# shidanxu/DistributedLPSolver

Hardware: AMD Instinct MI355X
Metric: simplex pivots/s + achieved HBM GB/s (dense fp64 tableau; roofline of the rank-64 tableau pass) (higher is better)
Workload: dtype f64

## Files before the change

distributedlpsolver_amd/csrc/dlp_defer.hip:

```cpp
#include <hip/hip_runtime.h>

#include <cmath>
#include <cstdlib>
#include <utility>

#include "dlp_internal.h"

namespace dlp {
namespace {

#include "dlp_device.h"

typedef unsigned int u4v __attribute__((ext_vector_type(4)));
typedef unsigned int u2v __attribute__((ext_vector_type(2)));
__device__ __forceinline__ u2v dbits(double v) {
    uint64_t u;
    __builtin_memcpy(&u, &v, sizeof(u));
    u2v w;
    w.x = (unsigned)u;
    w.y = (unsigned)(u >> 32);
    return w;
}

template <bool NT>
__device__ inline d2 ldv(const double* p) {
    if constexpr (NT)
        return __builtin_nontemporal_load((const d2*)p);
    else
        return *(const d2*)p;
}
template <bool NT>
__device__ inline double ldv1(const double* p) {
    if constexpr (NT)
        return __builtin_nontemporal_load(p);
    else
        return *p;
}
template <bool NT>
__device__ inline void stv1(double* p, double v) {
    if constexpr (NT)
        __builtin_nontemporal_store(v, p);
    else
        *p = v;
}
template <bool NT>
__device__ inline void stv(double* p, d2 v) {
    if constexpr (NT)
        __builtin_nontemporal_store(v, (d2*)p);
    else
        *(d2*)p = v;
}

__device__ __forceinline__ void glds16(const void* g, uint32_t m0) {
    asm volatile("s_waitcnt lgkmcnt(0)\n\tglobal_load_lds_dwordx4 %0, off" ::"v"(g), "{m0}"(m0) : "memory");
}
template <int N>
__device__ __forceinline__ void vmwait() { asm volatile("s_waitcnt vmcnt(%0)" ::"n"(N) : "memory"); }
__device__ __forceinline__ uint32_t lds_addr(const void* p) {
    return __builtin_amdgcn_readfirstlane((uint32_t)(uintptr_t)(const __attribute__((address_space(3))) void*)p);
}

constexpr int kAuxSc1 = 16;

__device__ inline void release_go(DevState* st) {
    __builtin_amdgcn_fence(__ATOMIC_RELEASE, "agent");
    asm volatile("s_waitcnt vmcnt(0)" ::: "memory");
    __hip_atomic_store(&st->go, 1u, __ATOMIC_RELAXED, __HIP_MEMORY_SCOPE_AGENT);
}

__device__ uint64_t g_chain_stamps[64][16];
__device__ int g_chain_stamps_on;
#define CHAIN_STAMP(slot, k)                                                                  \
    do {                                                                                      \
        if (g_chain_stamps_on && threadIdx.x == 0) g_chain_stamps[(slot) & 63][k] = wall_clock64(); \
    } while (0)
__device__ uint64_t g_wg_stamps[1024][8];
#define WG_STAMP(slot, k, v)                                                                   \
    do {                                                                                       \
        if (g_chain_stamps_on && threadIdx.x == 0 && ((slot) & 63) == 40 && blockIdx.x < 1024) \
            g_wg_stamps[blockIdx.x][k] = (v);                                                  \
    } while (0)

constexpr int kRatioRingPairs = 8;
constexpr size_t ratio_ring_bytes(int rp) { return (size_t)(kRatioDeferThreads / 64) * rp * 128 * sizeof(double); }
template <int KMAX, bool FUSED, bool LEAN = false, int LCH = 4, int RP = kRatioRingPairs, bool DB = false,
          int ROWS = 64, int RG = 1>
__device__ __forceinline__ void ratio_defer_body(
    const double* __restrict__ T, int64_t ld, int64_t rows, int64_t rows_elig, int64_t ncols,
    int64_t row_first, int32_t* basis, const PricePart* __restrict__ pp, int ntiles,
    DevState* st, double* __restrict__ C, int64_t ldc, double* __restrict__ Cc, int64_t ldcc,
    const double* __restrict__ P, double* __restrict__ rhs, int32_t* __restrict__ nzc,
    Cand* partials, Cand* cand_out, int nranks, double tol_dj, double tol_piv, int pricing,
    dlp_pivot* log, int64_t log_cap, int nblocks, const double* __restrict__ Ccp = nullptr,
    const double* __restrict__ Pp = nullptr, int prev_seal = -1, const XPeers* xp = nullptr,
    uint32_t xseq = 0, uint32_t* bcnt = nullptr, int brb = 1, int bnt = 0, const double* Tn = nullptr,
    int xsel = 0, uint32_t rseq = 0, Cond cd = Cond{}) {
    constexpr bool GRING = ROWS != 64 || RG != 1;
    constexpr int kPad = GRING ? 128 / ROWS * (RG + 1) : 0;
    constexpr int kWaves = GRING ? 16 : kRatioDeferThreads / 64;
    __shared__ PricePart lds_pp[kWaves];
    __shared__ Cand lds_c[kWaves];
    __shared__ int s_last;
    __shared__ double s_pq[KMAX + kPad], s_pn[KMAX];
    __shared__ int32_t s_pl[KMAX + kPad];
    auto cand_red = [&](Cand v) { return block_cand(v, lds_c); };
    const PricePart pp0 = (int)threadIdx.x < ntiles ? pp[threadIdx.x] : pp_empty();
    if (st->status != DLP_RUNNING) return;
// ... 1709 lines not shown
        vmwait<2 * U * (D - 1)>();
        return;
    }
    switch (g) {
        case 0: vmwait<U * (D - 1)>(); break;
        case 1: vmwait<U * (D - 1) + U>(); break;
        case 2: vmwait<U * (D - 1) + 2 * U>(); break;
        case 3: vmwait<U * (D - 1) + 3 * U>(); break;
        case 4: vmwait<U * (D - 1) + 4 * U>(); break;
        case 5: vmwait<U * (D - 1) + 5 * U>(); break;
        default: vmwait<U * (D - 1) + 6 * U>(); break;
    }
}
template <int U, int L>
__device__ __forceinline__ void ring_step(double (&t)[U], const double (&c)[U][2], const double (&pr)[64]) {
    constexpr int e = L & 1, n = (L & 31) >> 1;
#pragma unroll
    for (int u = 0; u < U; ++u) fmac_bc<n>(t[u], c[u][e], pr[L]);
}
template <int U, int L0, int... I>
__device__ __forceinline__ void ring_half(double (&t)[U], const double (&c)[U][2], const double (&pr)[64],
                                          std::integer_sequence<int, I...>) {
    (ring_step<U, L0 + I>(t, c, pr), ...);
}

template <int L>
__device__ __forceinline__ void redo_step(double& t, const double (&c)[2], const double (&pr)[64], int cl) {
    constexpr int e = L & 1, n = (L & 31) >> 1;
    if (L == cl)
        t = pr[L];
    else if (L > cl)
        fmac_bc<n>(t, c[e], pr[L]);
}
template <int L0, int... I>
__device__ __forceinline__ void redo_half(double& t, const double (&c)[2], const double (&pr)[64], int cl,
                                          std::integer_sequence<int, I...>) {
    (redo_step<L0 + I>(t, c, pr, cl), ...);
}
__device__ __forceinline__ double redo_pivot_row(const double* cr, int cl, const double (&pr)[64]) {
    int lane;
    asm volatile("v_mbcnt_lo_u32_b32 %0, -1, 0\n\tv_mbcnt_hi_u32_b32 %0, -1, %0" : "=v"(lane));
    double t = 0.0;
    if (cl < 32) {
        const d2 v = *(const d2*)(cr + 2 * (lane & 15));
        const double c0[2] = {v.x, v.y};
        redo_half<0>(t, c0, pr, cl, std::make_integer_sequence<int, 32>{});
    }
    const d2 v = *(const d2*)(cr + 32 + 2 * (lane & 15));
    const double c1[2] = {v.x, v.y};
    redo_half<32>(t, c1, pr, cl, std::make_integer_sequence<int, 32>{});
    return t;
}

template <bool NT, int U, int D, bool PUB = false>
__global__ __launch_bounds__(256) __attribute__((amdgpu_waves_per_eu(3))) void pass_q_kernel(
                                                     const double* __restrict__ T, double* __restrict__ Tout,
                                                     int64_t ld, int64_t rows, int64_t width,
                                                     const BlockDesc* __restrict__ bd,
                                                     const double* __restrict__ C, int64_t ldc,
                                                     const double* __restrict__ P,
                                                     const int32_t* __restrict__ nzc, int rb,
                                                     uint32_t* bcnt = nullptr, int pivg = 0) {
    constexpr int K = 64, SLOT = 128 * U;
    constexpr int kSt = (NT ? 2 : 0) | (PUB ? kAuxSc1 : 0);
    static_assert(U % 2 == 0, "one DMA carries two rows");
    __shared__ __attribute__((aligned(16))) int32_t cls[1024];
    typedef int32_t clsv __attribute__((ext_vector_type(U)));
    extern __shared__ double ring[];
    const int kb = bd->blk;
    const bool outplace = Tout != T;
    if (kb == 0 && !outplace) return;
    const int lane = threadIdx.x & 63;
    const int w = __builtin_amdgcn_readfirstlane(threadIdx.x >> 6);
    const int64_t j = (int64_t)blockIdx.x * 256 + threadIdx.x;
    const bool colok = j < width;
    const int jc = (int)(colok ? j : width - 1);
    double pr[K];
#pragma unroll
    for (int l = 0; l < K; ++l) pr[l] = P[(int64_t)l * ld + jc];
    const int64_t i0 = (int64_t)blockIdx.y * rb;
    const int64_t iend = (i0 + rb < rows) ? i0 + rb : rows;
    const int nr = (int)(iend - i0);
    classify_band(cls, bd, nzc, i0, nr, kb, pivg != 0);
    __syncthreads();
#pragma unroll
    for (int l = 0; l < K; ++l) asm volatile("" ::"v"(pr[l]));
    const int ng = (nr + U - 1) / U;
    const int64_t wc = (int64_t)blockIdx.x * 256 + w * 64 + 2 * (lane & 31);
    const int64_t wcc = wc < ld - 1 ? wc : ld - 2;
    const double* tsrc = T + i0 * ld + wcc;
    const double* csrc = C + i0 * ldc + 2 * (lane & 31);
    double* wbase = ring + (size_t)w * D * SLOT;
    const uint32_t lbase = (uint32_t)(uintptr_t)(const __attribute__((address_space(3))) void*)wbase;
    auto dma = [&](int g, int s) {
        const int gg = g < ng ? g : ng - 1;
#pragma unroll
        for (int k = 0; k < U / 2; ++k) {
            int r = gg * U + 2 * k + (lane >> 5);
            r = r < nr ? r : nr - 1;
            glds16(tsrc + (int64_t)r * ld, __builtin_amdgcn_readfirstlane(lbase + s * SLOT * 8 + k * 1024));
        }
#pragma unroll
        for (int k = 0; k < U / 2; ++k) {
            int r = gg * U + 2 * k + (lane >> 5);
            r = r < nr ? r : nr - 1;
            glds16(csrc + (int64_t)r * ldc,
                   __builtin_amdgcn_readfirstlane(lbase + s * SLOT * 8 + U * 512 + k * 1024));
        }
    };
    const int ld8 = (int)(ld * 8);
    const __amdgpu_buffer_rsrc_t ro = __builtin_amdgcn_make_buffer_rsrc(
        (void*)(Tout + i0 * ld), (short)0, (int)((int64_t)nr * ld * 8), 0x00020000);
    const int voff_st = colok ? jc * 8 : 0x7fffff00;
    auto store = [&](double v, int r, bool keep) {
        __builtin_amdgcn_raw_buffer_store_b64(__builtin_bit_cast(u2v, v), ro, keep ? voff_st : 0x7fffff00,
                                              (r < nr ? r : 0) * ld8, kSt);
    };
#pragma unroll
    for (int s = 0; s < D; ++s) dma(s, s);
    int s = 0;
    for (int g = 0; g < ng; ++g) {
        vmwait_group<D, U>(g);
        const double* sl = wbase + s * SLOT;
        const int r0 = g * U;
        const clsv cv = *(const clsv*)(cls + r0);
        bool dense = r0 + U <= nr, anyp = false;
#pragma unroll
        for (int u = 0; u < U; ++u) {
            const int cu = __builtin_amdgcn_readfirstlane(cv[u]);
            dense = dense && (cu == kDense || cu >= kDensePiv);
            anyp = anyp || cu >= kDensePiv;
        }
        if (dense) {
            double t[U];
#pragma unroll
            for (int u = 0; u < U; ++u) t[u] = sl[u * 64 + lane];
            double c[U][2];
            auto loadc = [&](int h) {
#pragma unroll
                for (int u = 0; u < U; ++u) {
                    const d2 v = *(const d2*)(sl + U * 64 + u * 64 + h * 32 + 2 * (lane & 15));
                    c[u][0] = v.x;
                    c[u][1] = v.y;
                }
            };
            loadc(0);
            ring_half<U, 0>(t, c, pr, std::make_integer_sequence<int, 32>{});
            loadc(1);
            ring_half<U, 32>(t, c, pr, std::make_integer_sequence<int, 32>{});
            if (anyp) {
#pragma nounroll
                for (int u = 0; u < U; ++u) {
                    const int cl = __builtin_amdgcn_readfirstlane(cls[r0 + u]) - kDensePiv;
                    if (cl < 0) continue;
                    const double tp = redo_pivot_row(sl + U * 64 + u * 64, cl, pr);
#pragma unroll
                    for (int k = 0; k < U; ++k) t[k] = k == u ? tp : t[k];
                }
            }
#pragma unroll
            for (int u = 0; u < U; ++u) store(t[u], r0 + u, true);
        } else {
            for (int u = 0; u < U; ++u) {
                const int r = r0 + u;
                int cl = r < nr ? cls[r] : kUntouched;
                if (cl >= kDensePiv) cl -= kDensePiv;
                double t = sl[u * 64 + lane];
                if (cl == kUntouched) {
                    store(t, r, outplace && r < nr);
                    continue;
                }
                const double* cr = sl + U * 64 + u * 64;
                t = replay_row(t, cl, pr, [&](int l) { return cr[l]; });
                store(t, r, true);
            }
        }
        dma(g + D, s);
        s = s + 1 == D ? 0 : s + 1;
    }
    if constexpr (PUB) {
        vmwait<0>();
        __syncthreads();
        if (threadIdx.x == 0) __hip_atomic_fetch_add(&bcnt[blockIdx.y], 1u, __ATOMIC_RELAXED, __HIP_MEMORY_SCOPE_AGENT);
    }
}


typedef double d4 __attribute__((ext_vector_type(4)));
template <bool NT_, int NT, bool PUB = false>
__global__ __launch_bounds__(256, 2) void pass_m_kernel(const double* __restrict__ T, double* __restrict__ Tout,
                                                     int64_t ld, int64_t rows, int64_t width,
                                                     const BlockDesc* __restrict__ bd,
                                                     const double* __restrict__ C, int64_t ldc,
                                                     const double* __restrict__ P,
                                                     const int32_t* __restrict__ nzc, int rb,
                                                     uint32_t* bcnt = nullptr) {
    constexpr int kSt = (NT_ ? 2 : 0) | (PUB ? kAuxSc1 : 0);
    constexpr int K = 64, KB = K / 4, W = 16 * NT, RS = K + 2;
    constexpr int NPC = (16 * RS + 127) / 128;
    __shared__ double lds_all[2 * NPC * 128 + 512];
    double(*As)[NPC * 128] = reinterpret_cast<double(*)[NPC * 128]>(lds_all);
    int32_t* cls = reinterpret_cast<int32_t*>(lds_all + 2 * NPC * 128);
    const int kb = bd->blk;
    const bool outplace = Tout != T;
    if (kb == 0 && !outplace) return;
    const int lane = threadIdx.x & 63;
    const int w = __builtin_amdgcn_readfirstlane(threadIdx.x >> 6);
    const int lr = lane & 15, lq = lane >> 4;
    const int64_t cw = (int64_t)blockIdx.x * (4 * W);
    const int64_t c0 = cw + w * W;
    double b[KB][NT];
#pragma unroll
    for (int k4 = 0; k4 < KB; ++k4)
#pragma unroll
        for (int t = 0; t < NT; ++t) {
            const int64_t col = c0 + 16 * t + lr;
            b[k4][t] = P[(int64_t)(4 * k4 + lq) * ld + (col < width ? col : width - 1)];
        }
    const int64_t i0 = (int64_t)blockIdx.y * rb;
    const int64_t iend = (i0 + rb < rows) ? i0 + rb : rows;
    const int nr = (int)(iend - i0);
    classify_band(cls, bd, nzc, i0, nr, kb);
    const int ng = (nr + 15) / 16;
    const int ld8 = (int)(ld * 8);
    const __amdgpu_buffer_rsrc_t ro = __builtin_amdgcn_make_buffer_rsrc(
        (void*)(Tout + i0 * ld), (short)0, (int)((int64_t)nr * ld * 8), 0x00020000);
    (void)ro;
    (void)ld8;
    auto stage = [&](int g, int buf) {
        const int gg = g < ng ? g : ng - 1;
// ... 93 lines not shown
                l = cl + 1;
            } else {
                t = row[j];
            }
            const double* cr = C + (i0 + r) * ldc;
            for (; l < kb; ++l) {
                const double f = cr[l];
                if (f != 0.0) t = __builtin_fma(-f, P[(int64_t)l * ld + j], t);
            }
        }
        if constexpr (PUB)
            __builtin_amdgcn_raw_buffer_store_b64(__builtin_bit_cast(u2v, t), ro, (int)j * 8 + r * ld8, 0, kSt);
        else
            Tout[(i0 + r) * ld + j] = t;
    }
    if constexpr (PUB) {
        asm volatile("s_waitcnt vmcnt(0)" ::: "memory");
        __syncthreads();
        if (threadIdx.x == 0) __hip_atomic_fetch_add(&bcnt[blockIdx.y], 1u, __ATOMIC_RELAXED, __HIP_MEMORY_SCOPE_AGENT);
    }
}

__global__ void blk_reset_kernel(DevState* st) {
    if (threadIdx.x == 0) {
        st->blk = 0;
        st->bser = st->bser + 1;
    }
}

__global__ __launch_bounds__(256) void reset_cols_kernel(double* __restrict__ T, int64_t ld, int64_t rows,
                                                         const int32_t* __restrict__ blkp,
                                                         const int32_t* __restrict__ pl,
                                                         const int32_t* __restrict__ qs) {
    const int64_t i = (int64_t)blockIdx.x * blockDim.x + threadIdx.x;
    if (i >= rows) return;
    const int kb = *blkp;
    double* r = T + i * ld;
    for (int l = 0; l < kb; ++l) r[qs[l]] = (pl[l] == (int32_t)i) ? 1.0 : 0.0;
}

__global__ __launch_bounds__(256) void drop_failed_step_kernel(const DevState* __restrict__ st,
                                                               const int32_t* __restrict__ blkp,
                                                               double* __restrict__ C, int64_t ldc,
                                                               int32_t* __restrict__ nzc, int64_t rows) {
    if (st->status != DLP_UNBOUNDED) return;
    const int kb = *blkp;
    const int64_t i = (int64_t)blockIdx.x * blockDim.x + threadIdx.x;
    if (i > rows || kb < 0 || kb >= ldc) return;
    const double a = C[i * ldc + kb];
    if (i < rows && a != 0.0) nzc[i] = nzc[i] - 1;
    C[i * ldc + kb] = 0.0;
}

__global__ __launch_bounds__(64) void seal_kernel(DevState* st, int slot, uint32_t* bcnt, int64_t nb) {
    const int kb = st->blk;
    for (int l = threadIdx.x; l < kMaxDefer; l += 64) {
        st->seal[slot].pl[l] = l < kb ? st->pl[l] : -1;
        st->seal[slot].qs[l] = st->qs[l];
    }
    if (bcnt)
        for (int64_t b = threadIdx.x; b < nb; b += 64) bcnt[b] = 0;
    __syncthreads();
    if (threadIdx.x == 0) {
        st->seal[slot].blk = kb;
        st->seal[slot].ser = st->bser;
        st->blk = 0;
        st->bser = st->bser + 1;
    }
}

}

static int ratio_ring_rows(const Geometry& g) {
    return g.rthreads >= 256 ? 64 : 0;
}

int ratio_defer_blocks(const Geometry& g) {
    return (int)((g.rows + 1 + g.rthreads - 1) / g.rthreads);
}
static int ratio_blocks_256(const Geometry& g) {
    return (int)((g.rows + 1 + kRatioDeferThreads - 1) / kRatioDeferThreads);
}

hipError_t launch_ratio_defer(const Geometry& g, const Defer& d, int32_t* basis,
                              const PricePart* pp, DevState* st, Cand* partials, int nblocks,
                              Cand* cand_out, int nranks, double tol_dj, double tol_piv,
                              int pricing, dlp_pivot* log, int64_t log_cap, hipStream_t s,
                              const Defer* prev, int prev_seal, const XPeers* xp, uint32_t xseq,
                              const BandPub* bp, bool xfuse, bool own_cus) {
    const int ntiles = (int)((g.width + kDeferTile - 1) / kDeferTile);
    const bool pub = bp && bp->cnt && bp->Tn && prev_seal >= 0;
    xfuse = xfuse && xp && nranks > 1;
    if (nblocks < ratio_defer_blocks(g)) return hipErrorInvalidValue;
    nblocks = ratio_defer_blocks(g);
    if (prev_seal >= 0 && (!prev || prev_seal > 1 || 2 * d.K > kMaxReplay)) return hipErrorInvalidValue;
    const double* Ccp = prev_seal >= 0 ? prev->Cc : nullptr;
    const double* Pp = prev_seal >= 0 ? prev->P : nullptr;
    const int steps = prev_seal >= 0 ? 2 * d.K : d.K;
    if (g.rthreads != 64 && g.rthreads != 128 && g.rthreads != 256) return hipErrorInvalidValue;
#define DLP_RATIO_DEFER(KM)                                                                      \
    ratio_defer_kernel<KM><<<nblocks, g.rthreads, 0, s>>>(                               \
        g.T, g.ld, g.rows, g.rows_elig, g.ncols, g.row_first, basis, pp, ntiles, st, d.C, d.ldc, \
        d.Cc, d.ldcc, d.P, d.rhs, d.nzc, partials, cand_out, nranks, tol_dj, tol_piv, pricing,   \
        log, log_cap, Ccp, Pp, prev_seal, xp, xseq, xfuse ? 1 : 0, g.cd)
    if (steps <= 8)
        DLP_RATIO_DEFER(8);
    else if (steps <= 16)
        DLP_RATIO_DEFER(16);
// ... 169 lines not shown
    g.T, g.ld, g.rows, g.rows_elig, g.ncols, g.nprice, g.row_first, basis, pp, ntiles, st, d.C, d.ldc, d.Cc, \
        d.ldcc, d.P, d.rhs, d.nzc, nrat, tol_dj, tol_piv, pricing, log, log_cap, Ccp, Pp, Cp, prev_seal, xp, \
        seq, pub ? bp->cnt + prev_seal * bp->stride : nullptr, pub ? bp->rb : 1, pub ? bp->ntiles : 0,     \
        pub ? bp->Tn : nullptr, 2, g.cd
    if (!ring && steps > 64 && g.cd.on) return hipErrorInvalidValue;
    if (ring) {
        if (g.rthreads == 128)
            pivot_x_ring_kernel<32><<<nrat + nprow, 256, (size_t)4 * 16 * 1024, s>>>(DLP_PX_ARGS);
        else
            pivot_x_ring_kernel<64><<<nrat + nprow, 256, (size_t)4 * 16 * 1024, s>>>(DLP_PX_ARGS);
    } else if (steps > 64)
        pivot_x_lean_kernel<<<nrat + nprow, 256, std::max(ratio_ring_bytes(kRatioRingPairs),
                                                          prow_ring_bytes(kProwRingSteps)), s>>>(DLP_PX_ARGS);
    else if (steps <= 16)
        pivot_x_kernel<16><<<nrat + nprow, 256, 0, s>>>(DLP_PX_ARGS);
    else if (steps <= 32)
        pivot_x_kernel<32><<<nrat + nprow, 256, 0, s>>>(DLP_PX_ARGS);
    else
        pivot_x_kernel<64><<<nrat + nprow, 256, 0, s>>>(DLP_PX_ARGS);
#undef DLP_PX_ARGS
    return hipGetLastError();
}

hipError_t launch_commit_defer(const Geometry& g, const Defer& d, DevState* st,
                               const int64_t* prow_bits, PricePart* pp, double tol_dj,
                               dlp_pivot* log, int64_t log_cap, hipStream_t s, const XPeers* xp,
                               uint32_t xseq) {
    const int blocks = (int)((g.ld + kDeferTile - 1) / kDeferTile);
    commit_defer_kernel<<<blocks, 256, 0, s>>>(g.T, g.ld, g.rows, g.ncols, g.nprice, st, d.C,
                                               d.ldc, d.P, prow_bits, pp, tol_dj, log, log_cap, xp,
                                               xseq, g.cd);
    return hipGetLastError();
}

template <bool NT, int K, int V, int U, int D>
static void launch_pass_r(const Geometry& g, const Defer& d, DevState* st, int rb, size_t dyn,
                          int order, hipStream_t s) {
    const int ntiles = (int)((g.width + 256 * V - 1) / (256 * V));
    const int nbands = (int)((g.rows + rb - 1) / rb);
    const int64_t total = (int64_t)ntiles * nbands;
    const int64_t t8 = (ntiles + 7) / 8;
    const dim3 grid((unsigned)(order == 1 ? 8 * ((total + 7) / 8) : order == 2 ? 8 * t8 * nbands : total));
    pass_r_kernel<NT, K, V, U, D, false><<<grid, 256, dyn, s>>>(
        g.T, g.ld, g.rows, g.width, st, d.C, d.ldc, d.P, d.nzc, rb, ntiles, nbands, order);
    pass_r_kernel<NT, K, V, U, D, true><<<grid, 256, dyn, s>>>(
        g.T, g.ld, g.rows, g.width, st, d.C, d.ldc, d.P, d.nzc, rb, ntiles, nbands, order);
}

static size_t pass_lds_env() {
    static const long v = std::getenv("DLP_PASS_LDS") ? std::atol(std::getenv("DLP_PASS_LDS")) : 0;
    return v > 0 && v <= 150 * 1024 ? (size_t)v : 0;
}

template <bool NT, int K>
static hipError_t pass(const Geometry& g, const Defer& d, DevState* st, int rb, int occ,
                       hipStream_t s, double* Tout, int seal, uint32_t* bcnt) {
    if (seal >= 0 && !lookahead_form(d.form)) return hipErrorInvalidValue;
    const BlockDesc* bd = seal >= 0 ? &st->seal[seal] : (const BlockDesc*)&st->blk;
    double* To = Tout ? Tout : g.T;
    if (d.form >= 6 && d.form <= 19 && d.form != 14 && d.form != 15 &&
        (int64_t)rb * g.ld * 8 < ((int64_t)1 << 31)) {
        if constexpr (K >= 16) {
            if ((d.form == 6 || d.form == 7 || d.form == 10 || d.form == 11 || d.form == 16 ||
                 d.form == 17) && K > 32)
                return hipErrorInvalidValue;
            size_t dyn = 0;
            if (occ > 0) {
                const size_t stat = 1024 * sizeof(int32_t) + 512 * sizeof(int16_t) + 16;
                dyn = (size_t)160 * 1024 / occ - stat;
            }
            if (g.rows > 0) {
                const int order = d.form <= 9 ? 1 : d.form <= 13 ? 0 : 2;
                const int f = d.form <= 9 ? d.form : d.form <= 13 ? d.form - 4 : d.form - 10;
                if (f == 6) {
                    if constexpr (K <= 32) launch_pass_r<NT, K, 2, 2, 4>(g, d, st, rb, dyn, order, s);
                } else if (f == 7) {
                    if constexpr (K <= 32) launch_pass_r<NT, K, 2, 2, 2>(g, d, st, rb, dyn, order, s);
                } else if (f == 8) {
                    launch_pass_r<NT, K, 1, 4, 4>(g, d, st, rb, dyn, order, s);
                } else {
                    launch_pass_r<NT, K, 1, 4, 2>(g, d, st, rb, dyn, order, s);
                }
            }
            blk_reset_kernel<<<1, 64, 0, s>>>(st);
            return hipGetLastError();
        }
    }
    if (d.form == 22 && K == 64 && d.K == 64 && d.ldc == 64 && rb <= 1024) {
        if constexpr (K == 64) {
            size_t dyn = 0;
            if (occ > 0) {
                const size_t stat = 1024 * sizeof(int32_t) + 2 * 9 * 128 * sizeof(double);
                dyn = (size_t)160 * 1024 / occ - stat;
            }
            const dim3 grid((unsigned)((g.width + 127) / 128), (unsigned)((g.rows + rb - 1) / rb));
            if (g.rows > 0) {
                if (bcnt && (int64_t)rb * g.ld * 8 < ((int64_t)1 << 31))
                    pass_m_kernel<NT, 2, true><<<grid, 256, dyn, s>>>(g.T, To, g.ld, g.rows, g.width, bd, d.C,
                                                                      d.ldc, d.P, d.nzc, rb, bcnt);
                else
                    pass_m_kernel<NT, 2><<<grid, 256, dyn, s>>>(g.T, To, g.ld, g.rows, g.width, bd, d.C, d.ldc,
                                                                 d.P, d.nzc, rb);
            }
            if (seal < 0) blk_reset_kernel<<<1, 64, 0, s>>>(st);
            return hipGetLastError();
        }
    }
    if (d.form == 21 && K == 64 && d.K == 64 && d.ldc == 64 && (int64_t)rb * g.ld * 8 < ((int64_t)1 << 31) &&
        (int64_t)rb * d.ldc * 8 < ((int64_t)1 << 31)) {
        if constexpr (K == 64) {
            size_t dyn = pass_lds_env();
            if (occ > 0) dyn = (size_t)160 * 1024 / occ - 1024 * sizeof(int32_t);
            const dim3 grid((unsigned)((g.width + 255) / 256), (unsigned)((g.rows + rb - 1) / rb));
            if (g.rows > 0) {
                if (bcnt)
                    pass_d_kernel<NT, true><<<grid, 256, dyn, s>>>(g.T, To, g.ld, g.rows, g.width, bd, d.C, d.ldc,
                                                                   d.P, d.nzc, rb, bcnt);
                else
                    pass_d_kernel<NT><<<grid, 256, dyn, s>>>(g.T, To, g.ld, g.rows, g.width, bd, d.C, d.ldc, d.P,
                                                             d.nzc, rb);
            }
            if (seal < 0) blk_reset_kernel<<<1, 64, 0, s>>>(st);
            return hipGetLastError();
        }
    }
    if (d.form == 23 && K == 64 && d.K == 64 && d.ldc == 64 && (int64_t)rb * g.ld * 8 < ((int64_t)1 << 31) &&
        rb <= 1024) {
        if constexpr (K == 64) {
            static const int qd = std::getenv("DLP_Q_DEPTH") ? std::atoi(std::getenv("DLP_Q_DEPTH")) : 4;
            static const int qu_env = std::getenv("DLP_Q_U") ? std::atoi(std::getenv("DLP_Q_U")) : 0;
            static const int pivg = std::getenv("DLP_PASS_PIVG") ? std::atoi(std::getenv("DLP_PASS_PIVG")) : 1;
            const int qu = qu_env == 2 || qu_env == 4 ? qu_env : (g.rows >= 16384 ? 4 : 2);
            constexpr int U = 2;
            const int D = qd == 2 || qd == 3 || qd == 6 || qd == 8 ? qd : 4;
            if (qu == 4) {
                const int D4 = qd == 3 ? 3 : 2;
                size_t dyn4 = std::max((size_t)4 * D4 * 128 * 4 * sizeof(double), pass_lds_env());
                if (occ > 0) dyn4 = std::max(dyn4, (size_t)160 * 1024 / occ - 1024 * sizeof(int32_t));
                const dim3 grid4((unsigned)((g.width + 255) / 256), (unsigned)((g.rows + rb - 1) / rb));
                if (g.rows > 0) {
                    if (D4 == 3) {
                        if (bcnt)
                            pass_q_kernel<NT, 4, 3, true><<<grid4, 256, dyn4, s>>>(g.T, To, g.ld, g.rows, g.width, bd,
                                                                                d.C, d.ldc, d.P, d.nzc, rb, bcnt, pivg);
                        else
                            pass_q_kernel<NT, 4, 3><<<grid4, 256, dyn4, s>>>(g.T, To, g.ld, g.rows, g.width, bd, d.C,
                                                                          d.ldc, d.P, d.nzc, rb, nullptr, pivg);
                    } else {
                        if (bcnt)
                            pass_q_kernel<NT, 4, 2, true><<<grid4, 256, dyn4, s>>>(g.T, To, g.ld, g.rows, g.width, bd,
                                                                                d.C, d.ldc, d.P, d.nzc, rb, bcnt, pivg);
                        else
                            pass_q_kernel<NT, 4, 2><<<grid4, 256, dyn4, s>>>(g.T, To, g.ld, g.rows, g.width, bd, d.C,
                                                                          d.ldc, d.P, d.nzc, rb, nullptr, pivg);
                    }
                }
                if (seal < 0) blk_reset_kernel<<<1, 64, 0, s>>>(st);
                return hipGetLastError();
            }
            size_t dyn = std::max((size_t)4 * D * 128 * U * sizeof(double), pass_lds_env());
            if (occ > 0) dyn = std::max(dyn, (size_t)160 * 1024 / occ - 1024 * sizeof(int32_t));
            const dim3 grid((unsigned)((g.width + 255) / 256), (unsigned)((g.rows + rb - 1) / rb));
#define DLP_PASS_Q(DD)                                                                                     \
    do {                                                                                                   \
        if (bcnt)                                                                                          \
            pass_q_kernel<NT, U, DD, true><<<grid, 256, dyn, s>>>(g.T, To, g.ld, g.rows, g.width, bd, d.C, \
                                                                  d.ldc, d.P, d.nzc, rb, bcnt, pivg);     \
        else                                                                                               \
            pass_q_kernel<NT, U, DD><<<grid, 256, dyn, s>>>(g.T, To, g.ld, g.rows, g.width, bd, d.C, d.ldc, \
                                                           d.P, d.nzc, rb, nullptr, pivg);                 \
    } while (0)
            if (g.rows > 0) {
                if (D == 2)
                    DLP_PASS_Q(2);
                else if (D == 3)
                    DLP_PASS_Q(3);
                else if (D == 6)
                    DLP_PASS_Q(6);
                else if (D == 8)
                    DLP_PASS_Q(8);
                else
                    DLP_PASS_Q(4);
            }
#undef DLP_PASS_Q
            if (seal < 0) blk_reset_kernel<<<1, 64, 0, s>>>(st);
            return hipGetLastError();
        }
    }
    const int form = (d.form >= 6 && d.form != 14 && d.form != 15 && d.form != 20) ? 3 : d.form;
    const int cols = (form == 0 || form == 4 || form >= 14) ? kDeferTile : 256;
    const int ntiles = (int)((g.width + cols - 1) / cols);
    const int64_t bands = (g.rows + rb - 1) / rb;
    size_t dyn = form >= 3 ? 0 : (size_t)K * rb * sizeof(double) + (size_t)rb * sizeof(int32_t);
    if (dyn > 160 * 1024) return hipErrorInvalidValue;
    if (occ > 0) {
        const size_t stat = form >= 14 ? 1024 * sizeof(int32_t) + 512 * sizeof(int16_t) + 16
                            : form >= 3 ? 1024 * sizeof(int32_t) : K * sizeof(int32_t);
        const size_t cap = (size_t)160 * 1024 / occ - stat;
        if (dyn < cap) dyn = cap;
    }
    const dim3 grid(ntiles, (unsigned)bands);
    const int tails = d.K == K ? 1 : 0;
    if (g.rows > 0) {
        if (form == 0) {
            if constexpr (K <= 32)
                pass_kernel<NT, K><<<grid, 256, dyn, s>>>(g.T, g.ld, g.rows, g.width, st, d.C,
                                                          d.ldc, d.P, rb);
            else
                return hipErrorInvalidValue;
        } else if (form == 3) {
            pass_s_kernel<NT, K, 1, 4, false><<<grid, 256, dyn, s>>>(g.T, To, g.ld, g.rows, g.width, bd,
                                                                     d.C, d.ldc, d.P, d.nzc, rb, tails);
            if (!tails)
                pass_s_kernel<NT, K, 1, 4, true><<<grid, 256, dyn, s>>>(g.T, To, g.ld, g.rows, g.width, bd,
                                                                        d.C, d.ldc, d.P, d.nzc, rb, 0);
        } else if (form == 20) {
            if constexpr (K <= 32) {
                pass_s_kernel<NT, K, 2, 2, false, true><<<grid, 256, dyn, s>>>(
                    g.T, To, g.ld, g.rows, g.width, bd, d.C, d.ldc, d.P, d.nzc, rb, tails);
                if (!tails)
                    pass_s_kernel<NT, K, 2, 2, true><<<grid, 256, dyn, s>>>(
                        g.T, To, g.ld, g.rows, g.width, bd, d.C, d.ldc, d.P, d.nzc, rb, 0);
            } else
                return hipErrorInvalidValue;
        } else if (form == 4 || form == 14 || form == 15) {
            if constexpr (K <= 32) {
                const int tl = (form == 14 || form == 15) ? 0 : tails;
                if (form == 15)
                    pass_s3_kernel<NT, K, 2, 2, false><<<grid, 256, dyn, s>>>(
                        g.T, To, g.ld, g.rows, g.width, bd, d.C, d.ldc, d.P, d.nzc, rb, tl);
                else
                    pass_s_kernel<NT, K, 2, 2, false><<<grid, 256, dyn, s>>>(
                        g.T, To, g.ld, g.rows, g.width, bd, d.C, d.ldc, d.P, d.nzc, rb, tl);
                if (form >= 14 && K >= 16 && (int64_t)rb * g.ld * 8 < ((int64_t)1 << 31)) {
                    const int nb = (int)bands;
// ... 5 lines not shown
                        g.T, To, g.ld, g.rows, g.width, bd, d.C, d.ldc, d.P, d.nzc, rb, 0);
                }
            } else
                return hipErrorInvalidValue;
        } else if (form == 5) {
            pass_s_kernel<NT, K, 1, 8, false><<<grid, 256, dyn, s>>>(g.T, To, g.ld, g.rows, g.width, bd,
                                                                     d.C, d.ldc, d.P, d.nzc, rb, tails);
            if (!tails)
                pass_s_kernel<NT, K, 1, 8, true><<<grid, 256, dyn, s>>>(g.T, To, g.ld, g.rows, g.width, bd,
                                                                        d.C, d.ldc, d.P, d.nzc, rb, 0);
        }
        else if (form == 1)
            pass1_kernel<NT, K, 2><<<grid, 256, dyn, s>>>(g.T, g.ld, g.rows, g.width, st, d.C,
                                                          d.ldc, d.P, rb);
        else
            pass1_kernel<NT, K, 4><<<grid, 256, dyn, s>>>(g.T, g.ld, g.rows, g.width, st, d.C,
                                                          d.ldc, d.P, rb);
    }
    if (seal < 0) blk_reset_kernel<<<1, 64, 0, s>>>(st);
    return hipGetLastError();
}

template <bool NT>
static hipError_t pass_k(const Geometry& g, const Defer& d, DevState* st, int rb, int occ,
                         hipStream_t s, double* Tout, int seal, uint32_t* bcnt) {
    if (d.K <= 4) return pass<NT, 4>(g, d, st, rb, occ, s, Tout, seal, nullptr);
    if (d.K <= 8) return pass<NT, 8>(g, d, st, rb, occ, s, Tout, seal, nullptr);
    if (d.K <= 16) return pass<NT, 16>(g, d, st, rb, occ, s, Tout, seal, nullptr);
    if (d.K <= 32) return pass<NT, 32>(g, d, st, rb, occ, s, Tout, seal, nullptr);
    return pass<NT, 64>(g, d, st, rb, occ, s, Tout, seal, bcnt);
}

bool lookahead_form(int form) {
    return form == 3 || form == 4 || form == 5 || form == 20 || form == 21 || form == 22 || form == 23;
}

int band_pub_tiles(int form, int64_t width) {
    return (int)(form == 22 ? (width + 127) / 128 : (width + 255) / 256);
}
bool band_pub_ok(const BandPub& bp, const Geometry& g, const Defer& d, int rb) {
    return (d.form == 21 || d.form == 22 || d.form == 23) && d.K == 64 && d.ldc == 64 && rb == bp.rb &&
           (g.rows + rb - 1) / rb <= bp.stride && band_pub_tiles(d.form, g.width) == bp.ntiles &&
           (int64_t)rb * g.ld * 8 < ((int64_t)1 << 31);
}

hipError_t launch_flush_defer(const Geometry& g, const Defer& d, DevState* st, bool nontemporal,
                              int rows_per_block, int occupancy, hipStream_t s, double* Tout,
                              int seal, const BandPub* bp) {
    if (d.K < 1 || d.K > kMaxDefer || rows_per_block < 1 || rows_per_block > 1024 || seal > 1)
        return hipErrorInvalidValue;
    uint32_t* bcnt = nullptr;
    if (bp && bp->cnt && seal >= 0 && Tout && Tout != g.T && band_pub_ok(*bp, g, d, rows_per_block))
        bcnt = bp->cnt + seal * bp->stride;
    if (g.rows > 0 && d.C && d.nzc) {
        drop_failed_step_kernel<<<(unsigned)((g.rows + 256) / 256), 256, 0, s>>>(
            st, seal >= 0 ? &st->seal[seal].blk : &st->blk, d.C, d.ldc, d.nzc, g.rows);
        const hipError_t e = hipGetLastError();
        if (e != hipSuccess) return e;
    }
    if (g.cd.on) {
        const hipError_t e = launch_reset_cols(g, st, seal, s);
        if (e != hipSuccess) return e;
    }
    return nontemporal ? pass_k<true>(g, d, st, rows_per_block, occupancy, s, Tout, seal, bcnt)
                       : pass_k<false>(g, d, st, rows_per_block, occupancy, s, Tout, seal, bcnt);
}

hipError_t chain_stamps_enable() {
    const int on = 1;
    return hipMemcpyToSymbol(HIP_SYMBOL(g_chain_stamps_on), &on, sizeof(on));
}
hipError_t chain_stamps_dump(uint64_t* host64x16) {
    return hipMemcpyFromSymbol(host64x16, HIP_SYMBOL(g_chain_stamps), sizeof(uint64_t) * 64 * 16);
}
hipError_t chain_wg_stamps_dump(uint64_t* host1024x8) {
    return hipMemcpyFromSymbol(host1024x8, HIP_SYMBOL(g_wg_stamps), sizeof(uint64_t) * 1024 * 8);
}

hipError_t launch_reset_cols(const Geometry& g, const DevState* st, int seal, hipStream_t s) {
    if (!g.cd.on || g.rows <= 0) return hipSuccess;
    const int32_t* blkp = seal >= 0 ? &st->seal[seal].blk : &st->blk;
    const int32_t* pl = seal >= 0 ? st->seal[seal].pl : st->pl;
    const int32_t* qs = seal >= 0 ? st->seal[seal].qs : st->qs;
    reset_cols_kernel<<<(unsigned)((g.rows + 255) / 256), 256, 0, s>>>(g.T, g.ld, g.rows, blkp, pl, qs);
    return hipGetLastError();
}

hipError_t launch_seal_defer(DevState* st, int slot, hipStream_t s, const BandPub* bp) {
    if (slot < 0 || slot > 1) return hipErrorInvalidValue;
    seal_kernel<<<1, 64, 0, s>>>(st, slot, bp && bp->cnt ? bp->cnt + slot * bp->stride : nullptr,
                                 bp ? bp->stride : 0);
    return hipGetLastError();
}

}
```

distributedlpsolver_amd/csrc/dlp_internal.h:

```cpp
#pragma once
#include <stddef.h>
#include <stdint.h>

#include <hip/hip_runtime.h>

#include "dlp.h"

namespace dlp {

constexpr int kUpdThreads = 256;
constexpr int kUpdVec = 2;
constexpr int kUpdTile = kUpdThreads * kUpdVec;
constexpr int kRatioThreads = 256;
constexpr int kRatioDeferThreads = 256;
constexpr int kProwThreads = 256;
constexpr int32_t kNoIndex = 0x7fffffff;
constexpr int kColqPad = 16;
constexpr int32_t kStatusSkip = 5;
constexpr int kMaxDefer = 64;
constexpr int kMaxReplay = 2 * kMaxDefer;
constexpr int kDeferTile = 512;

struct alignas(16) PricePart {
    double zmin;
// ... 139 lines not shown
hipError_t launch_xrow_recv(const XPeers* xp, uint32_t seq, int64_t ld, int64_t* out, DevState* st,
                            hipStream_t s);
int ratio_blocks(const Geometry& g);
int ratio_defer_blocks(const Geometry& g);
hipError_t launch_select(const Geometry& g, const Cand* cands, int nranks, int32_t* basis,
                         DevState* st, int pricing, dlp_pivot* log, int64_t log_cap,
                         hipStream_t s, bool forced = false, bool track = false,
                         const XPeers* xp = nullptr, uint32_t seq = 0);
hipError_t launch_cond_init(const Geometry& g, int64_t N, DevState* st, hipStream_t s);
hipError_t launch_reset_cols(const Geometry& g, const DevState* st, int seal, hipStream_t s);
hipError_t launch_drive(const Geometry& g, int64_t row, int32_t* basis, DevState* st,
                        double tol_piv, Cand* cand_out, int nranks, int pricing, dlp_pivot* log,
                        int64_t log_cap, double* colq, hipStream_t s);
hipError_t launch_gather_q(const Geometry& g, const DevState* st, double* colq, hipStream_t s);
hipError_t launch_carry_out(const Geometry& g, int64_t carry_local, int64_t* out, hipStream_t s);
hipError_t launch_carry_in(const Geometry& g, const int64_t* in, DevState* st, int pricing,
                           hipStream_t s);
hipError_t launch_set_status(DevState* st, int status, hipStream_t s);

hipError_t launch_ratio_defer(const Geometry& g, const Defer& d, int32_t* basis,
                              const PricePart* pp, DevState* st, Cand* partials, int nblocks,
                              Cand* cand_out, int nranks, double tol_dj, double tol_piv,
                              int pricing, dlp_pivot* log, int64_t log_cap, hipStream_t s,
                              const Defer* prev = nullptr, int prev_seal = -1,
                              const XPeers* xp = nullptr, uint32_t seq = 0, const BandPub* bp = nullptr,
                              bool xfuse = false, bool own_cus = false);
hipError_t launch_pivot_x(const Geometry& g, const Defer& d, int32_t* basis, PricePart* pp, DevState* st,
                          double tol_dj, double tol_piv, int pricing, dlp_pivot* log, int64_t log_cap,
                          hipStream_t s, const Defer* prev, int prev_seal, const XPeers* xp, uint32_t seq,
                          const BandPub* bp, bool own_cus = false);
int fused_pivot_blocks(const Geometry& g);
int fused_pivot_capacity(int K, int cus);
hipError_t launch_pivot_defer(const Geometry& g, const Defer& d, int32_t* basis, PricePart* pp,
                              DevState* st, Cand* partials, int nblocks, double tol_dj,
                              double tol_piv, int pricing, dlp_pivot* log, int64_t log_cap,
                              hipStream_t s);
hipError_t launch_prow_defer(const Geometry& g, const Defer& d, const DevState* st,
                             int64_t* prow_bits, PricePart* pp, double tol_dj, dlp_pivot* log,
                             int64_t log_cap, int nranks, hipStream_t s,
                             const Defer* prev = nullptr, int prev_seal = -1,
                             const XPeers* xp = nullptr, uint32_t seq = 0, const BandPub* bp = nullptr,
                             bool xfuse = false, bool own_cus = false);
hipError_t launch_commit_defer(const Geometry& g, const Defer& d, DevState* st,
                               const int64_t* prow_bits, PricePart* pp, double tol_dj,
                               dlp_pivot* log, int64_t log_cap, hipStream_t s,
                               const XPeers* xp = nullptr, uint32_t seq = 0);
hipError_t launch_flush_defer(const Geometry& g, const Defer& d, DevState* st, bool nontemporal,
                              int rows_per_block, int occupancy, hipStream_t s,
                              double* Tout = nullptr, int seal = -1, const BandPub* bp = nullptr);
bool lookahead_form(int form);
hipError_t chain_stamps_enable();
hipError_t chain_stamps_dump(uint64_t* host64x16);
hipError_t chain_wg_stamps_dump(uint64_t* host1024x8);
hipError_t launch_seal_defer(DevState* st, int slot, hipStream_t s, const BandPub* bp = nullptr);
hipError_t launch_prow(const Geometry& g, const DevState* st, int64_t* prow_bits, int nranks,
                       hipStream_t s);
hipError_t launch_update(const Geometry& g, const double* colq, const double* prow,
                         const DevState* st, PricePart* pp, double tol_dj, dlp_pivot* log,
                         int64_t log_cap, bool nontemporal, int variant, hipStream_t s);
size_t cluster_lds_bytes(int64_t m, int cw);
int cluster_plan(int64_t m, int64_t N, int max_wg, int* cw_out);
int64_t cluster_gstride(int64_t m);
int64_t cluster_granules(int64_t m, int nwg);
hipError_t launch_cluster(const Geometry& g, int64_t m, int64_t n, int nwg, int cw, DevState* st,
                          int32_t* basis, dlp_pivot* log, int64_t log_cap, uint64_t* gran,
                          int64_t max_pivots, int pricing, double tol_dj, double tol_piv,
                          hipStream_t s, uint64_t* stamps = nullptr);
hipError_t launch_generate(const Geometry& g, int kind, int64_t m, int64_t n, uint64_t seed,
                           hipStream_t s);
hipError_t launch_gather_column(const double* T, int64_t ld, int64_t nrows, int64_t col,
                                double* out, hipStream_t s);

hipError_t launch_reopt(const Geometry& g, int64_t n, int64_t N, const int32_t* rlist,
                        const double* cblist, int64_t R, const double* c, const int32_t* basic,
                        DevState* st, int pricing, hipStream_t s);

int dual_row_blocks(const Geometry& g);
int dual_col_blocks(const Geometry& g);
hipError_t launch_rhs_rebuild(const Geometry& g, int64_t n, const double* b, DevState* st, int pricing,
                              hipStream_t s);
hipError_t launch_dual_row(const Geometry& g, const int32_t* basis, DevState* st, Cand* partials,
                           double tol_feas, hipStream_t s);
hipError_t launch_dual_col(const Geometry& g, int32_t* basis, DevState* st, Cand* partials, double tol_piv,
                           int pricing, dlp_pivot* log, int64_t log_cap, hipStream_t s);

size_t batched_release(int device);

}
```

distributedlpsolver_amd/csrc/dlp_session.cpp:

```cpp
#include <hip/hip_runtime.h>
#include <rccl/rccl.h>

#include <algorithm>
#include <atomic>
#include <chrono>
#include <cmath>
#include <cstdio>
#include <cstdlib>
#include <cstring>
#include <mutex>
#include <new>
#include <string>
#include <thread>
#include <vector>

#include "dlp_host.h"
#include "dlp_internal.h"

namespace dlp {
static thread_local std::string g_err;
void set_error(const std::string& msg) { g_err = msg; }
}

using dlp::set_error;
// ... 918 lines not shown
}
int enqueue_prow(dlp_session* s) {
    HIP_TRY(dlp::launch_prow(s->g, s->st, s->prow_send, s->nranks, s->stream));
    return DLP_OK;
}
int enqueue_update(dlp_session* s) {
    const dlp_options& o = s->opt;
    HIP_TRY(dlp::launch_update(s->g, s->colq, (const double*)s->prow_recv, s->st, s->pp, o.tol_dj,
                               s->log, s->log_cap, o.nontemporal != 0, o.update_variant,
                               s->stream));
    return DLP_OK;
}

int enqueue_flush(dlp_session* s) {
    if (s->d.K <= 1) return DLP_OK;
    HIP_TRY(dlp::launch_flush_defer(s->g, s->d, s->st, s->opt.nontemporal != 0, s->defer_rb,
                                    s->defer_occ, s->stream));
    s->since_flush = 0;
    return DLP_OK;
}

int la_move_z(dlp_session* s, int to) {
    if (s->zbuf == to) return DLP_OK;
    HIP_TRY(hipMemcpyAsync(s->Tb[to] + s->rows * s->ld, s->Tb[s->zbuf] + s->rows * s->ld,
                           sizeof(double) * s->width, hipMemcpyDeviceToDevice, s->stream));
    s->zbuf = to;
    return DLP_OK;
}

int la_drain(dlp_session* s) {
    if (!s->la_pending) return DLP_OK;
    HIP_TRY(hipStreamWaitEvent(s->stream, s->ev_pass, 0));
    s->tread = s->tcur;
    s->la_pending = false;
    CALL_TRY(la_move_z(s, s->tread));
    s->T = s->g.T = s->Tb[s->tread];
    return DLP_OK;
}

dlp::BandPub band_pub(const dlp_session* s) {
    static const bool off = std::getenv("DLP_BAND_PUB") && std::atoi(std::getenv("DLP_BAND_PUB")) == 0;
    dlp::BandPub b;
    if (!s->band_cnt || off) return b;
    b.cnt = s->band_cnt;
    b.stride = s->band_stride;
    b.rb = s->defer_rb;
    b.ntiles = dlp::band_pub_tiles(s->d.form, s->g.width);
    b.Tn = s->la_pending ? s->Tb[s->tcur] : nullptr;
    return b;
}

int la_block_end(dlp_session* s, bool drain, hipEvent_t* evp) {
    const dlp::BandPub bp = band_pub(s);
    HIP_TRY(dlp::launch_seal_defer(s->st, s->cur, s->stream, &bp));
    HIP_TRY(hipEventRecord(s->ev_seal, s->stream));
    HIP_TRY(hipStreamWaitEvent(s->pstream, s->ev_seal, 0));
    if (evp) HIP_TRY(hipEventRecord(evp[0], s->pstream));
    dlp::Geometry gp = s->g;
    gp.T = s->Tb[s->tcur];
    HIP_TRY(dlp::launch_flush_defer(gp, s->dslot[s->cur], s->st, s->opt.nontemporal != 0, s->defer_rb,
                                    s->defer_occ, s->pstream, s->Tb[1 - s->tcur], s->cur, &bp));
    if (evp) HIP_TRY(hipEventRecord(evp[1], s->pstream));
    if (s->la_pending) HIP_TRY(hipStreamWaitEvent(s->stream, s->ev_pass, 0));
    HIP_TRY(hipEventRecord(s->ev_pass, s->pstream));
    s->tread = s->tcur;
    s->tcur = 1 - s->tcur;
    s->la_pending = true;
    s->cur = 1 - s->cur;
    s->since_flush = 0;
    CALL_TRY(la_move_z(s, s->tread));
    s->T = s->g.T = s->Tb[s->tread];
    if (drain) CALL_TRY(la_drain(s));
    return DLP_OK;
}

int la_disable(dlp_session* s) {
    if (!s->la) return DLP_OK;
    if (s->since_flush > 0) CALL_TRY(la_block_end(s, true, nullptr));
    CALL_TRY(la_drain(s));
    HIP_TRY(hipStreamSynchronize(s->stream));
    const int form = s->d.form;
    s->d = s->dslot[0];
    s->d.form = form;
    s->la = false;
    s->opt.lookahead = 0;
    CALL_TRY(chain_cus_apply(s, 0));
    pick_form(s);
    return DLP_OK;
}

int flush_pending_block(dlp_session* s) {
    if (!s->la && s->d.K > 1 && s->since_flush > 0) CALL_TRY(enqueue_flush(s));
    return DLP_OK;
}

bool rccl_lookahead_ok(const dlp_session* s) {
    if (s->nranks == 1) return true;
    const char* e = std::getenv("DLP_RCCL_LOOKAHEAD");
    return e && std::atoi(e) == 1;
}

int la_policy(dlp_session* s) {
    if (!s->la_auto || !s->exchange) return DLP_OK;
    const bool rccl_split = s->xmode == dlp_session::X_RCCL && rccl_lookahead_ok(s) && chain_cus_policy(s) > 0;
    const bool want = (s->xmode == dlp_session::X_PEER || rccl_split) && s->d.K == 64 && s->streaming &&
                      !s->general;
    if (want && !s->la) CALL_TRY(la_enable(s, false));
// ... 2251 lines not shown
```

Baseline: 14520.

## Use scalar-base DMA addressing in pass_q and fold failed-step drop into seal kernel

Adds an SA variant of pass_q_kernel that issues global_load_lds with a scalar base pointer and a fixed 32-bit vector offset. The base advances per row group, which removes per-lane 64-bit address arithmetic and row clamping from the steady-state DMA loop. It is enabled by default through DLP_PASS_SADDR. Separately, the failed-step column drop moves from a separate launch in the flush path into the single-wave seal kernel on the main stream, which removes one kernel launch from the pass stream. The catch is that the C column is now cleared serially by 64 threads, and an s_nop is inserted before each DMA.

New measurement: 14850, median of 6. +2.3%, better.

```diff
diff --git a/distributedlpsolver_amd/csrc/dlp_defer.hip b/distributedlpsolver_amd/csrc/dlp_defer.hip
--- a/distributedlpsolver_amd/csrc/dlp_defer.hip
+++ b/distributedlpsolver_amd/csrc/dlp_defer.hip
@@ -53,6 +53,10 @@
 
 __device__ __forceinline__ void glds16(const void* g, uint32_t m0) {
     asm volatile("s_waitcnt lgkmcnt(0)\n\tglobal_load_lds_dwordx4 %0, off" ::"v"(g), "{m0}"(m0) : "memory");
+}
+__device__ __forceinline__ void glds16s(uint32_t voff, const void* base, uint32_t m0) {
+    asm volatile("s_nop 4\n\ts_waitcnt lgkmcnt(0)\n\tglobal_load_lds_dwordx4 %0, %1" ::"v"(voff), "s"(base), "{m0}"(m0)
+                 : "memory");
 }
 template <int N>
 __device__ __forceinline__ void vmwait() { asm volatile("s_waitcnt vmcnt(%0)" ::"n"(N) : "memory"); }
@@ -1868,7 +1872,7 @@
     return t;
 }
 
-template <bool NT, int U, int D, bool PUB = false>
+template <bool NT, int U, int D, bool SA = false, bool PUB = false>
 __global__ __launch_bounds__(256) __attribute__((amdgpu_waves_per_eu(3))) void pass_q_kernel(
                                                      const double* __restrict__ T, double* __restrict__ Tout,
                                                      int64_t ld, int64_t rows, int64_t width,
@@ -1904,25 +1908,60 @@
     const int ng = (nr + U - 1) / U;
     const int64_t wc = (int64_t)blockIdx.x * 256 + w * 64 + 2 * (lane & 31);
     const int64_t wcc = wc < ld - 1 ? wc : ld - 2;
-    const double* tsrc = T + i0 * ld + wcc;
-    const double* csrc = C + i0 * ldc + 2 * (lane & 31);
     double* wbase = ring + (size_t)w * D * SLOT;
     const uint32_t lbase = (uint32_t)(uintptr_t)(const __attribute__((address_space(3))) void*)wbase;
+    uint32_t tvoff = 0, cvoff = 0;
+    const double *tsrc = nullptr, *csrc = nullptr;
+    if constexpr (SA) {
+        tvoff = (uint32_t)(lane >> 5) * (uint32_t)(ld * 8) + (uint32_t)(wcc * 8);
+        cvoff = 16u * lane;
+    } else {
+        tsrc = T + i0 * ld + wcc;
+        csrc = C + i0 * ldc + 2 * (lane & 31);
+    }
     auto dma = [&](int g, int s) {
         const int gg = g < ng ? g : ng - 1;
 #pragma unroll
         for (int k = 0; k < U / 2; ++k) {
-            int r = gg * U + 2 * k + (lane >> 5);
-            r = r < nr ? r : nr - 1;
-            glds16(tsrc + (int64_t)r * ld, __builtin_amdgcn_readfirstlane(lbase + s * SLOT * 8 + k * 1024));
+            const uint32_t m0 = __builtin_amdgcn_readfirstlane(lbase + s * SLOT * 8 + k * 1024);
+            if constexpr (SA) {
+                const int rk = gg * U + 2 * k;
+                const bool pair = rk + 1 < nr;
+                const uint32_t up = lane >> 5 ? (uint32_t)(ld * 8) : 0u;
+                glds16s(pair ? tvoff : tvoff - up, T + (i0 + (rk < nr ? rk : nr - 1)) * ld, m0);
+            } else {
+                int r = gg * U + 2 * k + (lane >> 5);
+                r = r < nr ? r : nr - 1;
+                glds16(tsrc + (int64_t)r * ld, m0);
+            }
         }
 #pragma unroll
         for (int k = 0; k < U / 2; ++k) {
-            int r = gg * U + 2 * k + (lane >> 5);
-            r = r < nr ? r : nr - 1;
-            glds16(csrc + (int64_t)r * ldc,
-                   __builtin_amdgcn_readfirstlane(lbase + s * SLOT * 8 + U * 512 + k * 1024));
-        }
+            const uint32_t m0 = __builtin_amdgcn_readfirstlane(lbase + s * SLOT * 8 + U * 512 + k * 1024);
+            if constexpr (SA) {
+                const int rk = gg * U + 2 * k;
+                const bool pair = rk + 1 < nr;
+                glds16s(pair ? cvoff : cvoff & 511u, C + (i0 + (rk < nr ? rk : nr - 1)) * ldc, m0);
+            } else {
+                int r = gg * U + 2 * k + (lane >> 5);
+                r = r < nr ? r : nr - 1;
+                glds16(csrc + (int64_t)r * ldc, m0);
+            }
+        }
+    };
+    const int ngs = SA ? nr / U : 0;
+    const int64_t tstep = (int64_t)U * ld * 8, cstep = (int64_t)U * ldc * 8;
+    const char* tb = (const char*)(T + i0 * ld) + D * tstep;
+    const char* cb = (const char*)(C + i0 * ldc) + D * cstep;
+    auto dma_s = [&](int s) {
+#pragma unroll
+        for (int k = 0; k < U / 2; ++k)
+            glds16s(tvoff, tb + (int64_t)2 * k * ld * 8,
+                    __builtin_amdgcn_readfirstlane(lbase + s * SLOT * 8 + k * 1024));
+#pragma unroll
+        for (int k = 0; k < U / 2; ++k)
+            glds16s(cvoff, cb + (int64_t)2 * k * ldc * 8,
+                    __builtin_amdgcn_readfirstlane(lbase + s * SLOT * 8 + U * 512 + k * 1024));
     };
     const int ld8 = (int)(ld * 8);
     const __amdgpu_buffer_rsrc_t ro = __builtin_amdgcn_make_buffer_rsrc(
@@ -1991,7 +2030,15 @@
                 store(t, r, true);
             }
         }
-        dma(g + D, s);
+        if (SA && g + D < ngs) {
+            dma_s(s);
+        } else {
+            dma(g + D, s);
+        }
+        if constexpr (SA) {
+            tb += tstep;
+            cb += cstep;
+        }
         s = s + 1 == D ? 0 : s + 1;
     }
     if constexpr (PUB) {
@@ -2191,8 +2238,16 @@
     C[i * ldc + kb] = 0.0;
 }
 
-__global__ __launch_bounds__(64) void seal_kernel(DevState* st, int slot, uint32_t* bcnt, int64_t nb) {
+__global__ __launch_bounds__(64) void seal_kernel(DevState* st, int slot, uint32_t* bcnt, int64_t nb,
+                                                  double* __restrict__ C, int64_t ldc,
+                                                  int32_t* __restrict__ nzc, int64_t rows) {
     const int kb = st->blk;
+    if (C && nzc && st->status == DLP_UNBOUNDED && kb >= 0 && kb < ldc)
+        for (int64_t i = threadIdx.x; i <= rows; i += 64) {
+            const double a = C[i * ldc + kb];
+            if (i < rows && a != 0.0) nzc[i] = nzc[i] - 1;
+            C[i * ldc + kb] = 0.0;
+        }
     for (int l = threadIdx.x; l < kMaxDefer; l += 64) {
         st->seal[slot].pl[l] = l < kb ? st->pl[l] : -1;
         st->seal[slot].qs[l] = st->qs[l];
@@ -2468,6 +2523,14 @@
     return v > 0 && v <= 150 * 1024 ? (size_t)v : 0;
 }
 
+static bool pass_q_runs(const Geometry& g, const Defer& d, int rb) {
+    return d.form == 23 && d.K == 64 && d.ldc == 64 && (int64_t)rb * g.ld * 8 < ((int64_t)1 << 31) && rb <= 1024;
+}
+static bool pass_saddr_env() {
+    static const int v = std::getenv("DLP_PASS_SADDR") ? std::atoi(std::getenv("DLP_PASS_SADDR")) : 1;
+    return v != 0;
+}
+
 template <bool NT, int K>
 static hipError_t pass(const Geometry& g, const Defer& d, DevState* st, int rb, int occ,
                        hipStream_t s, double* Tout, int seal, uint32_t* bcnt) {
@@ -2540,63 +2603,57 @@
             return hipGetLastError();
         }
     }
-    if (d.form == 23 && K == 64 && d.K == 64 && d.ldc == 64 && (int64_t)rb * g.ld * 8 < ((int64_t)1 << 31) &&
-        rb <= 1024) {
+    if (K == 64 && pass_q_runs(g, d, rb)) {
         if constexpr (K == 64) {
             static const int qd = std::getenv("DLP_Q_DEPTH") ? std::atoi(std::getenv("DLP_Q_DEPTH")) : 4;
             static const int qu_env = std::getenv("DLP_Q_U") ? std::atoi(std::getenv("DLP_Q_U")) : 0;
             static const int pivg = std::getenv("DLP_PASS_PIVG") ? std::atoi(std::getenv("DLP_PASS_PIVG")) : 1;
+            const bool sad = pass_saddr_env();
             const int qu = qu_env == 2 || qu_env == 4 ? qu_env : (g.rows >= 16384 ? 4 : 2);
             constexpr int U = 2;
             const int D = qd == 2 || qd == 3 || qd == 6 || qd == 8 ? qd : 4;
+            const dim3 grid((unsigned)((g.width + 255) / 256), (unsigned)((g.rows + rb - 1) / rb));
+#define DLP_PASS_Q(UU, DD, DYN)                                                                                \
+    do {                                                                                                       \
+        if (bcnt && sad)                                                                                       \
+            pass_q_kernel<NT, UU, DD, true, true><<<grid, 256, DYN, s>>>(g.T, To, g.ld, g.rows, g.width, bd, d.C, \
+                                                                         d.ldc, d.P, d.nzc, rb, bcnt, pivg);  \
+        else if (bcnt)                                                                                         \
+            pass_q_kernel<NT, UU, DD, false, true><<<grid, 256, DYN, s>>>(g.T, To, g.ld, g.rows, g.width, bd, d.C, \
+                                                                          d.ldc, d.P, d.nzc, rb, bcnt, pivg); \
+        else if (sad)                                                                                          \
+            pass_q_kernel<NT, UU, DD, true, false><<<grid, 256, DYN, s>>>(g.T, To, g.ld, g.rows, g.width, bd, d.C, \
+                                                                          d.ldc, d.P, d.nzc, rb, nullptr, pivg); \
+        else                                                                                                   \
+            pass_q_kernel<NT, UU, DD, false, false><<<grid, 256, DYN, s>>>(g.T, To, g.ld, g.rows, g.width, bd, d.C, \
+                                                                           d.ldc, d.P, d.nzc, rb, nullptr, pivg); \
+    } while (0)
             if (qu == 4) {
                 const int D4 = qd == 3 ? 3 : 2;
                 size_t dyn4 = std::max((size_t)4 * D4 * 128 * 4 * sizeof(double), pass_lds_env());
                 if (occ > 0) dyn4 = std::max(dyn4, (size_t)160 * 1024 / occ - 1024 * sizeof(int32_t));
-                const dim3 grid4((unsigned)((g.width + 255) / 256), (unsigned)((g.rows + rb - 1) / rb));
                 if (g.rows > 0) {
-                    if (D4 == 3) {
-                        if (bcnt)
-                            pass_q_kernel<NT, 4, 3, true><<<grid4, 256, dyn4, s>>>(g.T, To, g.ld, g.rows, g.width, bd,
-                                                                                d.C, d.ldc, d.P, d.nzc, rb, bcnt, pivg);
-                        else
-                            pass_q_kernel<NT, 4, 3><<<grid4, 256, dyn4, s>>>(g.T, To, g.ld, g.rows, g.width, bd, d.C,
-                                                                          d.ldc, d.P, d.nzc, rb, nullptr, pivg);
-                    } else {
-                        if (bcnt)
-                            pass_q_kernel<NT, 4, 2, true><<<grid4, 256, dyn4, s>>>(g.T, To, g.ld, g.rows, g.width, bd,
-                                                                                d.C, d.ldc, d.P, d.nzc, rb, bcnt, pivg);
-                        else
-                            pass_q_kernel<NT, 4, 2><<<grid4, 256, dyn4, s>>>(g.T, To, g.ld, g.rows, g.width, bd, d.C,
-                                                                          d.ldc, d.P, d.nzc, rb, nullptr, pivg);
-                    }
+                    if (D4 == 3)
+                        DLP_PASS_Q(4, 3, dyn4);
+                    else
+                        DLP_PASS_Q(4, 2, dyn4);
                 }
                 if (seal < 0) blk_reset_kernel<<<1, 64, 0, s>>>(st);
                 return hipGetLastError();
             }
             size_t dyn = std::max((size_t)4 * D * 128 * U * sizeof(double), pass_lds_env());
             if (occ > 0) dyn = std::max(dyn, (size_t)160 * 1024 / occ - 1024 * sizeof(int32_t));
-            const dim3 grid((unsigned)((g.width + 255) / 256), (unsigned)((g.rows + rb - 1) / rb));
-#define DLP_PASS_Q(DD)                                                                                     \
-    do {                                                                                                   \
-        if (bcnt)                                                                                          \
-            pass_q_kernel<NT, U, DD, true><<<grid, 256, dyn, s>>>(g.T, To, g.ld, g.rows, g.width, bd, d.C, \
-                                                                  d.ldc, d.P, d.nzc, rb, bcnt, pivg);     \
-        else                                                                                               \
-            pass_q_kernel<NT, U, DD><<<grid, 256, dyn, s>>>(g.T, To, g.ld, g.rows, g.width, bd, d.C, d.ldc, \
-                                                           d.P, d.nzc, rb, nullptr, pivg);                 \
-    } while (0)
             if (g.rows > 0) {
                 if (D == 2)
-                    DLP_PASS_Q(2);
+                    DLP_PASS_Q(U, 2, dyn);
                 else if (D == 3)
-                    DLP_PASS_Q(3);
+                    DLP_PASS_Q(U, 3, dyn);
                 else if (D == 6)
-                    DLP_PASS_Q(6);
+                    DLP_PASS_Q(U, 6, dyn);
                 else if (D == 8)
-                    DLP_PASS_Q(8);
+                    DLP_PASS_Q(U, 8, dyn);
                 else
-                    DLP_PASS_Q(4);
+                    DLP_PASS_Q(U, 4, dyn);
             }
 #undef DLP_PASS_Q
             if (seal < 0) blk_reset_kernel<<<1, 64, 0, s>>>(st);
@@ -2708,9 +2765,9 @@
     uint32_t* bcnt = nullptr;
     if (bp && bp->cnt && seal >= 0 && Tout && Tout != g.T && band_pub_ok(*bp, g, d, rows_per_block))
         bcnt = bp->cnt + seal * bp->stride;
-    if (g.rows > 0 && d.C && d.nzc) {
-        drop_failed_step_kernel<<<(unsigned)((g.rows + 256) / 256), 256, 0, s>>>(
-            st, seal >= 0 ? &st->seal[seal].blk : &st->blk, d.C, d.ldc, d.nzc, g.rows);
+    if (seal < 0 && g.rows > 0 && d.C && d.nzc) {
+        drop_failed_step_kernel<<<(unsigned)((g.rows + 256) / 256), 256, 0, s>>>(st, &st->blk, d.C, d.ldc, d.nzc,
+                                                                                g.rows);
         const hipError_t e = hipGetLastError();
         if (e != hipSuccess) return e;
     }
@@ -2742,10 +2799,12 @@
     return hipGetLastError();
 }
 
-hipError_t launch_seal_defer(DevState* st, int slot, hipStream_t s, const BandPub* bp) {
+hipError_t launch_seal_defer(const Geometry& g, const Defer& d, DevState* st, int slot, hipStream_t s,
+                             const BandPub* bp) {
     if (slot < 0 || slot > 1) return hipErrorInvalidValue;
+    const bool drop = g.rows > 0 && d.C && d.nzc;
     seal_kernel<<<1, 64, 0, s>>>(st, slot, bp && bp->cnt ? bp->cnt + slot * bp->stride : nullptr,
-                                 bp ? bp->stride : 0);
+                                 bp ? bp->stride : 0, drop ? d.C : nullptr, d.ldc, drop ? d.nzc : nullptr, g.rows);
     return hipGetLastError();
 }
 
diff --git a/distributedlpsolver_amd/csrc/dlp_internal.h b/distributedlpsolver_amd/csrc/dlp_internal.h
--- a/distributedlpsolver_amd/csrc/dlp_internal.h
+++ b/distributedlpsolver_amd/csrc/dlp_internal.h
@@ -215,7 +215,8 @@
 hipError_t chain_stamps_enable();
 hipError_t chain_stamps_dump(uint64_t* host64x16);
 hipError_t chain_wg_stamps_dump(uint64_t* host1024x8);
-hipError_t launch_seal_defer(DevState* st, int slot, hipStream_t s, const BandPub* bp = nullptr);
+hipError_t launch_seal_defer(const Geometry& g, const Defer& d, DevState* st, int slot, hipStream_t s,
+                             const BandPub* bp = nullptr);
 hipError_t launch_prow(const Geometry& g, const DevState* st, int64_t* prow_bits, int nranks,
                        hipStream_t s);
 hipError_t launch_update(const Geometry& g, const double* colq, const double* prow,
diff --git a/distributedlpsolver_amd/csrc/dlp_session.cpp b/distributedlpsolver_amd/csrc/dlp_session.cpp
--- a/distributedlpsolver_amd/csrc/dlp_session.cpp
+++ b/distributedlpsolver_amd/csrc/dlp_session.cpp
@@ -994,7 +994,7 @@
 
 int la_block_end(dlp_session* s, bool drain, hipEvent_t* evp) {
     const dlp::BandPub bp = band_pub(s);
-    HIP_TRY(dlp::launch_seal_defer(s->st, s->cur, s->stream, &bp));
+    HIP_TRY(dlp::launch_seal_defer(s->g, s->dslot[s->cur], s->st, s->cur, s->stream, &bp));
     HIP_TRY(hipEventRecord(s->ev_seal, s->stream));
     HIP_TRY(hipStreamWaitEvent(s->pstream, s->ev_seal, 0));
     if (evp) HIP_TRY(hipEventRecord(evp[0], s->pstream));
```
